# lucidrains/imagen-pytorch

Hardware: AMD Instinct MI355X
Metric: images/sec (64->256 cascade, 1000 steps, bs=8) (higher is better)
Workload: dtype f16; 1 GPU; C3: README unet1 (dim 32, 64^2) + unet2 (dim 32, 256^2, lowres_cond) cascade, 1000 DDPM steps/stage, CFG 3.0, dynamic thresholding, batch 8 per GPU; global_batch=8, parallelism=batch-sharded x1, one RCCL all-gather of final images, batch_schedule=5 whole cascades side by side (one stream each), images_in_flight=40, denoiser_evals_per_image=4000

## Files before the change

imagen-pytorch_amd/_abi.py:

```python
from __future__ import annotations

import ctypes
import os
import re
from typing import Dict

HERE = os.path.dirname(os.path.abspath(__file__))
ROOT = os.path.dirname(HERE)
HEADER = os.path.join(ROOT, "include", "imagen_hip.h")
LIB_PATH = os.environ.get("IMAGEN_LIB_PATH") or os.path.join(HERE, "libimagen_hip.so")

KNOWN_ENV = {"IMAGEN_LIB_PATH", "IMAGEN_TIMING", "IMAGEN_TIME_TABLE", "IMAGEN_TIME_TABLE_MAX_GB", "IMAGEN_CONV_PRO", "IMAGEN_CONV_GEMM",
             "IMAGEN_CONV_SMALL", "IMAGEN_ROWCHAIN", "IMAGEN_EMUL_TESTS", "IMAGEN_BENCH_LANES", "IMAGEN_BENCH_MODE", "IMAGEN_VIDEO_GPU_TESTS"}
_stale = sorted(k for k in os.environ if k.startswith("IMAGEN_") and k not in KNOWN_ENV)
if _stale:
    raise RuntimeError(f"{', '.join(_stale)}: not read by this version (switches of earlier rounds are module constants of imagen_pytorch_amd.ops / "
                       f".engine now: monkeypatch them); known variables: {', '.join(sorted(KNOWN_ENV))}")

_CTYPE = {
    "int32_t": ctypes.c_int32,
    "uint32_t": ctypes.c_uint32,
    "uint8_t": ctypes.c_uint8,
    "float": ctypes.c_float,
}


def _parse_header(path: str):
    text = open(path).read()
    text = re.sub(r"/\*.*?\*/", "", text, flags=re.S)
    text = re.sub(r"//[^\n]*", "", text)
    enums: Dict[str, int] = {}
    for m in re.finditer(r"enum\s*\w*\s*\{(.*?)\}", text, flags=re.S):
        nxt = 0
        for item in m.group(1).split(","):
            item = item.strip()
            if not item:
                continue
            if "=" in item:
                name, val = [s.strip() for s in item.split("=")]
                nxt = int(val, 0)
            else:
                name = item
            enums[name] = nxt
            nxt += 1
    for m in re.finditer(r"#define\s+(IMAGEN_\w+)\s+\(?([0-9x*+ ]+)\)?\s*$", text, flags=re.M):
        try:
            enums[m.group(1)] = int(eval(m.group(2), {}, {}))
        except Exception:
            pass
    structs = {}
    for m in re.finditer(r"typedef\s+struct\s+(\w+)\s*\{(.*?)\}\s*(\w+)\s*;", text, flags=re.S):
        name, body = m.group(3), m.group(2)
        fields = []
        for decl in body.split(";"):
            decl = " ".join(decl.split())
            if not decl:
                continue
            if "*" in decl:
                fname = decl.split("*")[-1].strip()
                fields.append((fname, ctypes.c_void_p))
            else:
                parts = decl.split(" ", 1)
                ctype = _CTYPE[parts[0]]
                for fname in parts[1].split(","):
                    fields.append((fname.strip(), ctype))
        structs[name] = fields
    return enums, structs


ENUMS, _STRUCT_FIELDS = _parse_header(HEADER)


def _make_struct(name, fields):
    return type(name, (ctypes.Structure,), {"_fields_": fields})


STRUCTS = {name: _make_struct(name, fields) for name, fields in _STRUCT_FIELDS.items()}
globals().update(STRUCTS)

OP_STRUCT = {
    ENUMS["IMAGEN_OP_IGEMM"]: STRUCTS["ImagenIgemmParams"],
    ENUMS["IMAGEN_OP_ROWSTAT"]: STRUCTS["ImagenRowstatParams"],
    ENUMS["IMAGEN_OP_ATTENTION"]: STRUCTS["ImagenAttentionParams"],
    ENUMS["IMAGEN_OP_KV_PREP"]: STRUCTS["ImagenKvPrepParams"],
    ENUMS["IMAGEN_OP_QNORM"]: STRUCTS["ImagenQnormParams"],
    ENUMS["IMAGEN_OP_GCA_PARTIAL"]: STRUCTS["ImagenGcaPartialParams"],
    ENUMS["IMAGEN_OP_GCA_FINAL"]: STRUCTS["ImagenGcaFinalParams"],
    ENUMS["IMAGEN_OP_GATE_RESIDUAL"]: STRUCTS["ImagenGateResidualParams"],
    ENUMS["IMAGEN_OP_LN_RESIDUAL"]: STRUCTS["ImagenLnResidualParams"],
    ENUMS["IMAGEN_OP_TIME_EMBED"]: STRUCTS["ImagenTimeEmbedParams"],
    ENUMS["IMAGEN_OP_SCALE_SHIFT"]: STRUCTS["ImagenScaleShiftParams"],
    ENUMS["IMAGEN_OP_PACK_IMAGE"]: STRUCTS["ImagenPackImageParams"],
    ENUMS["IMAGEN_OP_CFG_X0"]: STRUCTS["ImagenCfgX0Params"],
    ENUMS["IMAGEN_OP_QUANTILE"]: STRUCTS["ImagenQuantileParams"],
    ENUMS["IMAGEN_OP_DDPM_UPDATE"]: STRUCTS["ImagenDdpmUpdateParams"],
    ENUMS["IMAGEN_OP_ROWS_COPY"]: STRUCTS["ImagenRowsCopyParams"],
    ENUMS["IMAGEN_OP_MEMSET32"]: STRUCTS["ImagenMemset32Params"],
    ENUMS["IMAGEN_OP_SELECT_ROWS"]: STRUCTS["ImagenSelectRowsParams"],
    ENUMS["IMAGEN_OP_MEAN_ROWS"]: STRUCTS["ImagenMeanRowsParams"],
    ENUMS["IMAGEN_OP_RANDN"]: STRUCTS["ImagenRandnParams"],
    ENUMS["IMAGEN_OP_LOWRES_PREP"]: STRUCTS["ImagenLowresPrepParams"],
    ENUMS["IMAGEN_OP_LINCOMB"]: STRUCTS["ImagenLincombParams"],
    ENUMS["IMAGEN_OP_KV_PREP_MULTI"]: STRUCTS["ImagenKvPrepMultiParams"],
    ENUMS["IMAGEN_OP_TEMPORAL_PEG"]: STRUCTS["ImagenTemporalPegParams"],
    ENUMS["IMAGEN_OP_TEMPORAL_ATTENTION"]: STRUCTS["ImagenTemporalAttentionParams"],
    ENUMS["IMAGEN_OP_ACT_PREP"]: STRUCTS["ImagenActPrepParams"],
    ENUMS["IMAGEN_OP_GCA_TAIL"]: STRUCTS["ImagenGcaTailParams"],
    ENUMS["IMAGEN_OP_STEP_SLICE"]: STRUCTS["ImagenStepSliceParams"],
    ENUMS["IMAGEN_OP_ROWCHAIN"]: STRUCTS["ImagenRowchainParams"],
    ENUMS["IMAGEN_OP_LINEAR_F32"]: STRUCTS["ImagenLinearF32Params"],
    ENUMS["IMAGEN_OP_LINCTX"]: STRUCTS["ImagenLinCtxParams"],
    ENUMS["IMAGEN_OP_LINEAR_XATTN"]: STRUCTS["ImagenLinearXattnParams"],
}
STRUCT_KIND = {v: k for k, v in OP_STRUCT.items()}

EXPORTED_SYMBOLS = [
    "imagen_abi_version", "imagen_last_error", "imagen_sizeof", "imagen_launch", "imagen_plan_run",
    "imagen_igemm_num_configs", "imagen_igemm_config_info", "imagen_igemm_stage_slots", "imagen_igemm_config_family", "imagen_igemm_config_ring", "imagen_igemm_lds_bytes", "imagen_igemm_packed_elems", "imagen_pack_igemm_weights",
    "imagen_graph_begin", "imagen_graph_end", "imagen_graph_launch", "imagen_graph_destroy",
    "imagen_event_create", "imagen_event_record", "imagen_event_elapsed_ms", "imagen_event_destroy",
    "imagen_probe_copy", "imagen_probe_mfma", "imagen_probe_latency", "imagen_probe_launch_chain",
]


class ImagenHipError(RuntimeError):
    pass


_lib = None


def load_library(path: str = LIB_PATH) -> ctypes.CDLL:
    global _lib
    if _lib is not None:
        return _lib
    if not os.path.exists(path):
        raise ImagenHipError(
            f"{path} not found: the HIP extension is the product path and has no fallback. "
            "Build it with `python -c 'import __graft_entry__ as g; g.build()'` (needs hipcc)."
        )
    import torch

    lib = ctypes.CDLL(path)
    for sym in EXPORTED_SYMBOLS:
        if not hasattr(lib, sym):
            raise ImagenHipError(f"{path} does not export {sym}")
    lib.imagen_last_error.restype = ctypes.c_char_p
    lib.imagen_sizeof.restype = ctypes.c_size_t
    lib.imagen_sizeof.argtypes = [ctypes.c_int]
    lib.imagen_launch.argtypes = [ctypes.c_int, ctypes.c_void_p, ctypes.c_size_t, ctypes.c_void_p]
    lib.imagen_plan_run.argtypes = [ctypes.c_void_p, ctypes.c_int, ctypes.c_void_p]
    lib.imagen_igemm_config_info.argtypes = [ctypes.c_int] + [ctypes.POINTER(ctypes.c_int)] * 3
    lib.imagen_igemm_stage_slots.argtypes = [ctypes.c_int] * 3
    lib.imagen_igemm_config_family.argtypes = [ctypes.c_int]
    lib.imagen_igemm_config_ring.argtypes = [ctypes.c_int]
    lib.imagen_igemm_lds_bytes.restype = ctypes.c_long
    lib.imagen_igemm_lds_bytes.argtypes = [ctypes.c_int] * 6
    lib.imagen_igemm_packed_elems.restype = ctypes.c_size_t
    lib.imagen_igemm_packed_elems.argtypes = [ctypes.c_int] * 5
    lib.imagen_pack_igemm_weights.argtypes = [ctypes.c_int, ctypes.c_void_p, ctypes.c_void_p] + [ctypes.c_int] * 5 + [ctypes.c_void_p]
    lib.imagen_graph_begin.argtypes = [ctypes.c_void_p]
    lib.imagen_graph_end.argtypes = [ctypes.c_void_p, ctypes.POINTER(ctypes.c_void_p)]
    lib.imagen_graph_launch.argtypes = [ctypes.c_void_p, ctypes.c_void_p]
    lib.imagen_graph_destroy.argtypes = [ctypes.c_void_p]
    lib.imagen_event_create.argtypes = [ctypes.POINTER(ctypes.c_void_p)]
    lib.imagen_event_record.argtypes = [ctypes.c_void_p, ctypes.c_void_p]
    lib.imagen_event_elapsed_ms.argtypes = [ctypes.c_void_p, ctypes.c_void_p, ctypes.POINTER(ctypes.c_float)]
    lib.imagen_event_destroy.argtypes = [ctypes.c_void_p]
    lib.imagen_probe_copy.argtypes = [ctypes.c_void_p, ctypes.c_void_p, ctypes.c_size_t, ctypes.c_int, ctypes.c_void_p, ctypes.POINTER(ctypes.c_float)]
    lib.imagen_probe_mfma.argtypes = [ctypes.c_int, ctypes.c_int, ctypes.c_void_p, ctypes.c_void_p, ctypes.POINTER(ctypes.c_float)]
    lib.imagen_probe_latency.argtypes = [ctypes.c_void_p, ctypes.c_int, ctypes.c_void_p, ctypes.c_void_p, ctypes.POINTER(ctypes.c_float)]
    lib.imagen_probe_launch_chain.argtypes = [ctypes.c_int, ctypes.c_int, ctypes.c_void_p, ctypes.c_void_p, ctypes.POINTER(ctypes.c_float)]
    if lib.imagen_abi_version() != ENUMS["IMAGEN_ABI_VERSION"]:
        raise ImagenHipError("libimagen_hip.so ABI version does not match include/imagen_hip.h")
    for kind, st in OP_STRUCT.items():
        if lib.imagen_sizeof(kind) != ctypes.sizeof(st):
            raise ImagenHipError(f"struct size mismatch for op kind {kind}: C {lib.imagen_sizeof(kind)} vs ctypes {ctypes.sizeof(st)}")
    _lib = lib
    return lib


def hip_runtime_copies() -> list:
    seen = []
    try:
        with open("/proc/self/maps") as f:
            for line in f:
                if "libamdhip64" in line:
                    path = line.split()[-1]
                    if path not in seen:
                        seen.append(path)
    except OSError:
        pass
    return seen


def check(rc: int, what: str = "") -> None:
    if rc != 0:
        msg = load_library().imagen_last_error().decode(errors="replace")
        raise ImagenHipError(f"{what or 'libimagen_hip'} failed (rc={rc}): {msg}")


class OpRef(ctypes.Structure):
    _fields_ = [("kind", ctypes.c_int32), ("params_bytes", ctypes.c_int32), ("params", ctypes.c_void_p)]
```

imagen-pytorch_amd/build_ext.py:

```python
from __future__ import annotations

import hashlib
import os
import shutil
import subprocess
import sys

HERE = os.path.dirname(os.path.abspath(__file__))
ROOT = os.path.dirname(HERE)
CSRC = os.path.join(HERE, "csrc")
SOURCES = ["igemm.hip", "conv_dma.hip", "conv_stream.hip", "conv_pw.hip", "conv_big.hip", "conv_pro.hip", "conv_gemm.hip", "conv_small.hip", "rowchain.hip", "elementwise.hip", "attention.hip", "sampler.hip", "temporal.hip", "linear_xattn.hip", "codesize.hip", "probe.hip", "capi.hip"]
LIB = os.path.join(HERE, "libimagen_hip.so")
STAMP = os.path.join(HERE, ".libimagen_hip.stamp")


def _torch_lib_dir():
    try:
        import torch
        return os.path.join(os.path.dirname(torch.__file__), "lib")
    except Exception:
        return None


def _digest() -> str:
    h = hashlib.sha256()
    for name in sorted(os.listdir(CSRC)):
        with open(os.path.join(CSRC, name), "rb") as f:
            h.update(name.encode())
            h.update(f.read())
    with open(os.path.join(ROOT, "include", "imagen_hip.h"), "rb") as f:
        h.update(f.read())
    return h.hexdigest()


def build(force: bool = False, verbose: bool = True) -> str:
    digest = _digest()
    if not force and os.path.exists(LIB) and os.path.exists(STAMP) and open(STAMP).read().strip() == digest:
        return LIB
    hipcc = shutil.which("hipcc") or "/opt/rocm/bin/hipcc"
    if not os.path.exists(hipcc):
        raise RuntimeError("hipcc not found: cannot build libimagen_hip.so")
    objs = []
    build_dir = os.path.join(HERE, "build")
    os.makedirs(build_dir, exist_ok=True)
    common = [hipcc, "--offload-arch=gfx950", "-O3", "-std=c++17", "-fPIC", "-I" + os.path.join(ROOT, "include"), "-I" + CSRC]
    procs = []
    for src in SOURCES:
        obj = os.path.join(build_dir, src.replace(".hip", ".o"))
        objs.append(obj)
        procs.append((src, subprocess.Popen(common + ["-c", os.path.join(CSRC, src), "-o", obj],
                                            stdout=subprocess.PIPE, stderr=subprocess.STDOUT)))
    for src, pr in procs:
        out, _ = pr.communicate()
        if pr.returncode != 0:
            raise RuntimeError(f"hipcc failed on {src}:\n{out.decode()}")
        if verbose and out.strip():
            print(out.decode())
    link = [hipcc, "--offload-arch=gfx950", "-shared", "-fPIC", "-o", LIB] + objs
    tl = _torch_lib_dir()
    if tl and os.path.exists(os.path.join(tl, "libamdhip64.so")):
        link += ["-L" + tl, "-Wl,-rpath," + tl]
    link += ["-Wl,-rpath,/opt/rocm/lib"]
    res = subprocess.run(link, stdout=subprocess.PIPE, stderr=subprocess.STDOUT)
    if res.returncode != 0:
        raise RuntimeError("link failed:\n" + res.stdout.decode())
    with open(STAMP, "w") as f:
        f.write(digest)
    if verbose:
        print(f"built {LIB}")
    return LIB


def build_variant(tag: str, defs, sources=None) -> str:
    hipcc = shutil.which("hipcc") or "/opt/rocm/bin/hipcc"
    build_dir = os.path.join(HERE, "build", tag)
    os.makedirs(build_dir, exist_ok=True)
    common = [hipcc, "--offload-arch=gfx950", "-O3", "-std=c++17", "-fPIC", "-I" + os.path.join(ROOT, "include"), "-I" + CSRC] + list(defs)
    procs, objs = [], []
    for src in SOURCES:
        obj = os.path.join(build_dir, src.replace(".hip", ".o"))
        objs.append(obj)
        procs.append((src, subprocess.Popen(common + ["-c", os.path.join(CSRC, src), "-o", obj], stdout=subprocess.PIPE, stderr=subprocess.STDOUT)))
    for src, pr in procs:
        out, _ = pr.communicate()
        if pr.returncode != 0:
            raise RuntimeError(f"hipcc failed on {src}:\n{out.decode()}")
    lib = os.path.join(HERE, f"libimagen_hip_{tag}.so")
    link = [hipcc, "--offload-arch=gfx950", "-shared", "-fPIC", "-o", lib] + objs
    tl = _torch_lib_dir()
    if tl and os.path.exists(os.path.join(tl, "libamdhip64.so")):
        link += ["-L" + tl, "-Wl,-rpath," + tl]
    link += ["-Wl,-rpath,/opt/rocm/lib"]
    res = subprocess.run(link, stdout=subprocess.PIPE, stderr=subprocess.STDOUT)
    if res.returncode != 0:
        raise RuntimeError("link failed:\n" + res.stdout.decode())
    return lib


if __name__ == "__main__":
    build(force="--force" in sys.argv)
```

imagen-pytorch_amd/csrc/conv_families.h:

```cpp
#pragma once
#include "common.h"

int imagen_conv_dma_num_configs();
int imagen_conv_dma_config_info(int idx, int* tile_pixels, int* tile_cout, int* kgroups);
long imagen_conv_dma_lds_bytes(int idx, int KH, int KW, int TH, int TW);
int launch_conv_dma(const ImagenIgemmParams* p, int idx, hipStream_t s);
int imagen_conv_dma_ring(int idx);
int imagen_conv_stream_num_configs();
int imagen_conv_stream_config_info(int idx, int* tile_pixels, int* tile_cout, int* kgroups);
long imagen_conv_stream_lds_bytes(int idx, int KH, int KW, int TH, int TW);
int launch_conv_stream(const ImagenIgemmParams* p, int idx, hipStream_t s);
int imagen_conv_pw_num_configs();
int imagen_conv_pw_config_info(int idx, int* tile_pixels, int* tile_cout, int* kgroups);
long imagen_conv_pw_lds_bytes(int idx, int KH, int KW, int TH, int TW);
int launch_conv_pw(const ImagenIgemmParams* p, int idx, hipStream_t s);
int imagen_conv_big_num_configs();
int imagen_conv_big_config_info(int idx, int* tile_pixels, int* tile_cout, int* kgroups);
long imagen_conv_big_lds_bytes(int idx, int KH, int KW, int TH, int TW);
int launch_conv_big(const ImagenIgemmParams* p, int idx, hipStream_t s);
int imagen_conv_pro_num_configs();
int imagen_conv_pro_config_info(int idx, int* tile_pixels, int* tile_cout, int* kgroups);
long imagen_conv_pro_lds_bytes(int idx, int KH, int KW, int TH, int TW);
int launch_conv_pro(const ImagenIgemmParams* p, int idx, hipStream_t s);
int imagen_conv_gemm_num_configs();
int imagen_conv_gemm_config_info(int idx, int* tile_pixels, int* tile_cout, int* kgroups);
long imagen_conv_gemm_lds_bytes(int idx, int KH, int KW, int TH, int TW);
int launch_conv_gemm(const ImagenIgemmParams* p, int idx, hipStream_t s);
int imagen_conv_small_num_configs();
int imagen_conv_small_config_info(int idx, int* tile_pixels, int* tile_cout, int* kgroups);
long imagen_conv_small_lds_bytes(int idx, int KH, int KW, int TH, int TW);
int launch_conv_small(const ImagenIgemmParams* p, int idx, hipStream_t s);

struct ConvFamily {
  int id;
  int (*num)();
  int (*info)(int idx, int* tile_pixels, int* tile_cout, int* kgroups);
  long (*lds)(int idx, int KH, int KW, int TH, int TW);
  int (*launch)(const ImagenIgemmParams* p, int idx, hipStream_t s);
  int kh, kw;
  int (*ring)(int idx);
};
```

imagen-pytorch_amd/csrc/igemm.hip:

```cpp
#include <algorithm>
#include <cstdio>
#include <cstdlib>
#include <type_traits>
#include <utility>
#include "common.h"
#include "conv_families.h"

namespace {

struct TileCfg { int MI, NI, WM, WN, G; };
constexpr int kBiasLds = 1024;

constexpr int stage_slots(int TP, int G, int KSC) {
  if (KSC == 18 && G == 4) return TP == 64 ? 2 : TP == 128 ? 3 : 6;
  if (KSC == 2 && G == 4) return TP / 64;
  if (KSC == 8 && G == 4) return TP == 64 ? 4 : 6;
  if (KSC == 6 && G == 4) return TP == 64 ? 3 : TP == 128 ? 4 : 5;
  if (KSC == 4 && G == 8) return TP / 32;
  if (KSC == 8 && G == 16) return TP / 16;
  return 4;
}

constexpr TileCfg kCfgs[] = {
    {2, 1, 4, 1, 4},
// ... 603 lines not shown
          if (p.act_out == IMAGEN_ACT_SILU) {
#pragma unroll
            for (int e = 0; e < 4; ++e) v[e] = silu_f(v[e]);
          } else if (p.act_out == IMAGEN_ACT_GELU) {
#pragma unroll
            for (int e = 0; e < 4; ++e) v[e] = gelu_f(v[e]);
          }
          if (p.out_mode == IMAGEN_OUT_NCHW_F32) {
            float* y = reinterpret_cast<float*>(p.y);
#pragma unroll
            for (int e = 0; e < 4; ++e)
              if (co + e < p.Cout) y[((size_t)b * p.Cout + co + e) * (p.OH * p.OW) + op[mi]] = v[e];
            continue;
          }
          if (addend) {
            const f16x4 ad = cur.ar[mi];
            v[0] += (float)ad[0] * cur.g.x; v[1] += (float)ad[1] * cur.g.y; v[2] += (float)ad[2] * cur.g.z; v[3] += (float)ad[3] * cur.g.w;
          } else if (res) {
            const f16x4 rr = cur.ar[mi];
#pragma unroll
            for (int e = 0; e < 4; ++e) v[e] += (float)rr[e];
          }
          f16x4 o;
#pragma unroll
          for (int e = 0; e < 4; ++e) {
            o[e] = (f16)v[e];
            const float r = (float)o[e];
            ssq_px[mi] += r * r;
          }
          outv[ni][q][mi] = o;
        }
      } else {
#pragma unroll
        for (int mi = 0; mi < MI; ++mi) outv[ni][q][mi] = f16x4{};
      }
    });
    prime_weights(n0_next);
    if (wide) {
      f16* y = reinterpret_cast<f16*>(p.y) + (size_t)b * p.bsy;
#pragma unroll
      for (int ni = 0; ni < NI; ++ni)
#pragma unroll
        for (int qp = 0; qp < 2; ++qp) {
          const int cx = n0 + (wn * NI + ni) * 32 + 8 * qp + 16 * half;
#pragma unroll
          for (int mi = 0; mi < MI; ++mi) {
            const imagen_u32x4 v = imagen_pair_quads(outv[ni][qp][mi], outv[ni][qp + 2][mi]);
            if (cx < p.Cout && op[mi] >= 0) *reinterpret_cast<imagen_u32x4*>(y + (size_t)op[mi] * p.ldy + cx) = v;
          }
        }
    } else if (wide_ps) {
      f16* y = reinterpret_cast<f16*>(p.y) + (size_t)b * p.bsy;
      const int Cq = p.Cout >> 2;
#pragma unroll
      for (int ni = 0; ni < NI; ++ni)
#pragma unroll
        for (int qp = 0; qp < 2; ++qp) {
          const int cx = n0 + (wn * NI + ni) * 32 + 8 * qp + 16 * half;
          const int sub = cx / Cq, c = cx - sub * Cq;
#pragma unroll
          for (int mi = 0; mi < MI; ++mi) {
            const imagen_u32x4 v = imagen_pair_quads(outv[ni][qp][mi], outv[ni][qp + 2][mi]);
            const int oy = tc.oy0 + pix_y[mi], ox = tc.ox0 + pix_x[mi];
            const int yy = 2 * oy + (sub >> 1), xx = 2 * ox + (sub & 1);
            if (cx < p.Cout && op[mi] >= 0) *reinterpret_cast<imagen_u32x4*>(y + ((size_t)yy * (2 * p.OW) + xx) * p.ldy + c) = v;
          }
        }
    } else if (p.out_mode != IMAGEN_OUT_NCHW_F32) {
      f16* y = reinterpret_cast<f16*>(p.y);
#pragma unroll
      for (int ni = 0; ni < NI; ++ni)
#pragma unroll
        for (int q = 0; q < 4; ++q) {
          const int co = n0 + (wn * NI + ni) * 32 + 8 * q + 4 * half;
          if (co >= p.Cout) continue;
#pragma unroll
          for (int mi = 0; mi < MI; ++mi) {
            if (op[mi] < 0) continue;
            if (p.out_mode == IMAGEN_OUT_PIXEL_SHUFFLE) {
              const int Cq = p.Cout >> 2;
              const int sub = co / Cq, c = co - sub * Cq;
              const int oy = tc.oy0 + pix_y[mi], ox = tc.ox0 + pix_x[mi];
              const int yy = 2 * oy + (sub >> 1), xx = 2 * ox + (sub & 1);
              *reinterpret_cast<f16x4*>(y + (size_t)b * p.bsy + ((size_t)yy * (2 * p.OW) + xx) * p.ldy + c) = outv[ni][q][mi];
            } else {
              *reinterpret_cast<f16x4*>(y + (size_t)b * p.bsy + (size_t)op[mi] * p.ldy + co) = outv[ni][q][mi];
            }
          }
        }
    }
    }
    if (p.ssq_out) {
#pragma unroll
      for (int mi = 0; mi < MI; ++mi) ssq_px[mi] += __shfl_xor(ssq_px[mi], 32);
      if (WN == 1) {
        if (half == 0) {
#pragma unroll
          for (int mi = 0; mi < MI; ++mi) {
            const int oy = tc.oy0 + pix_y[mi], ox = tc.ox0 + pix_x[mi];
            if (oy < p.OH && ox < p.OW) p.ssq_out[(size_t)b * (p.OH * p.OW) + oy * p.OW + ox] = ssq_px[mi];
          }
        }
      } else {
        if (half == 0) {
#pragma unroll
          for (int mi = 0; mi < MI; ++mi) ep_red[(wm * WN + wn) * PXW + mi * 32 + l31] = ssq_px[mi];
        }
        lds_barrier();
        if (wn == 0 && half == 0) {
#pragma unroll
          for (int mi = 0; mi < MI; ++mi) {
            float tot = 0.0f;
#pragma unroll
            for (int w = 0; w < WN; ++w) tot += ep_red[(wm * WN + w) * PXW + mi * 32 + l31];
            const int oy = tc.oy0 + pix_y[mi], ox = tc.ox0 + pix_x[mi];
            if (oy < p.OH && ox < p.OW) p.ssq_out[(size_t)b * (p.OH * p.OW) + oy * p.OW + ox] = tot;
          }
        }
      }
    }
  };

  TileCoord tc = decode(t_cursor);
  prime_weights(tc.n0);
  unsigned warm_ep = 0;
  if constexpr (GEN) {
    const f16* eop = addend ? addend + (size_t)tc.b * p.bs_add : (res ? res + (size_t)tc.b * p.bs_res : nullptr);
    const int eld = addend ? p.ld_add : p.ld_res;
    if (eop) {
#pragma unroll
      for (int mi = 0; mi < MI; ++mi) {
        const int oy = tc.oy0 + pix_y[mi], ox = tc.ox0 + pix_x[mi];
        const int opx = (oy < p.OH && ox < p.OW) ? oy * p.OW + ox : 0;
#pragma unroll
        for (int ni = 0; ni < NI; ++ni) {
          const int co = min(tc.n0 + (wn * NI + ni) * 32 + 4 * half, p.Cout - 4);
          warm_ep ^= *reinterpret_cast<const volatile unsigned*>(eop + (size_t)opx * eld + co);
        }
      }
      if (addend) warm_ep ^= *reinterpret_cast<const volatile unsigned*>(p.gate + (size_t)tc.b * p.gate_stride + min(tc.n0 + wn * NI * 32 + (lane & 31), p.Cout - 1));
    }
  }
  lds_barrier();
  imagen_code_warm_sink(warm);
  imagen_code_warm_sink(warm_ep);
  int cur = 0;
  while (true) {
    const int t_next = t_cursor + t_step;
    const int n0_next = t_next < t_end ? decode(t_next).n0 : tc.n0;
    for (int chunk = 0; chunk < NC; ++chunk) {
      compute(smem + cur * buf_bytes);
      lds_barrier();
      cur ^= 1;
    }
    epilogue(tc, n0_next);
    if (t_next >= t_end) break;
    zero_acc();
    t_cursor = t_next;
    tc = decode(t_cursor);
  }
}

inline int num_cus() {
  static int n = 0;
  if (n == 0) {
    int dev = 0, v = 0;
    if (hipGetDevice(&dev) == hipSuccess && hipDeviceGetAttribute(&v, hipDeviceAttributeMultiprocessorCount, dev) == hipSuccess && v > 0) n = v;
    else n = 256;
  }
  return n;
}

template <int MI, int NI, int WM, int WN, int G, int KSC, bool GEN>
int launch_gen(const ImagenIgemmParams& p, hipStream_t s);

template <int MI, int NI, int WM, int WN, int G, int KSC>
int launch_ksc(const ImagenIgemmParams& p, hipStream_t s) {
  const bool plain = p.act_out == IMAGEN_ACT_NONE && p.out_mode == IMAGEN_OUT_NHWC && !p.addend && !p.res &&
                     (p.bias == nullptr || p.Cout_pad <= kBiasLds);
  return plain ? launch_gen<MI, NI, WM, WN, G, KSC, false>(p, s) : launch_gen<MI, NI, WM, WN, G, KSC, true>(p, s);
}

template <int MI, int NI, int WM, int WN, int G, int KSC, bool GEN>
int launch_gen(const ImagenIgemmParams& p, hipStream_t s) {
  constexpr int TP = 32 * MI * WM, BN = 32 * NI * WN;
  const int ITW = (p.TW - 1) * p.stride + p.KW, ITH = (p.TH - 1) * p.stride + p.KH;
  const int IT = ITH * ITW;
  IMAGEN_CHECK(p.TH * p.TW == TP, "igemm: tile %dx%d does not match cfg %d (%d pixels)", p.TH, p.TW, p.cfg, TP);
  IMAGEN_CHECK(IT * G <= stage_slots(TP, G, KSC) * 256, "igemm: halo tile too large (%d px x %d groups > %d staging slots)", IT, G,
               stage_slots(TP, G, KSC));
  IMAGEN_CHECK(p.Cout_pad % BN == 0, "igemm: Cout_pad %d not a multiple of %d", p.Cout_pad, BN);
  IMAGEN_CHECK(p.Cin_pad % (8 * G) == 0, "igemm: Cin_pad %d not a multiple of %d", p.Cin_pad, 8 * G);
  IMAGEN_CHECK(p.C1 % 8 == 0 && p.C2 % 8 == 0 && p.ld1 % 8 == 0 && (p.x2 == nullptr || p.ld2 % 8 == 0),
               "igemm: channel counts / strides must be multiples of 8 (C1=%d C2=%d ld1=%d ld2=%d)", p.C1, p.C2, p.ld1, p.ld2);
  IMAGEN_CHECK(p.out_mode == IMAGEN_OUT_NCHW_F32 || p.Cout % 4 == 0, "igemm: Cout %d must be a multiple of 4", p.Cout);
  IMAGEN_CHECK(p.out_mode != IMAGEN_OUT_PIXEL_SHUFFLE || p.Cout % 16 == 0, "igemm: pixel-shuffle needs Cout %% 16 == 0");
  IMAGEN_CHECK(!p.post_pa || (p.post_ps && p.out_mode == IMAGEN_OUT_NHWC && p.Cout <= BN && !p.addend && !p.res && !p.ssq_out &&
                              p.act_out == IMAGEN_ACT_NONE && p.Cout % 4 == 0),
               "igemm: post_pa needs post_ps, a plain NHWC output and one workgroup covering all %d output channels (tile has %d)", p.Cout, BN);
  IMAGEN_CHECK(!(p.addend && p.res), "igemm: addend and residual are mutually exclusive");
  IMAGEN_CHECK(!p.ssq_out || (p.out_mode == IMAGEN_OUT_NHWC && p.Cout <= BN),
               "igemm: ssq_out needs NHWC output and one workgroup covering all %d output channels (tile has %d)", p.Cout, BN);
  const size_t lds = (size_t)2 * IT * Geo<G>::PS + (size_t)(4 * 32 * MI + kBiasLds) * sizeof(float) + 16;
  IMAGEN_CHECK(lds <= 160 * 1024, "igemm: LDS tile %zu bytes too large", lds);
  auto kern = igemm_kernel<MI, NI, WM, WN, G, KSC, GEN>;
  static bool attr_done[16] = {};
  int dev = 0;
  (void)hipGetDevice(&dev);
  if (dev < 0 || dev >= 16 || !attr_done[dev]) {
    hipError_t e = hipFuncSetAttribute(reinterpret_cast<const void*>(kern), hipFuncAttributeMaxDynamicSharedMemorySize, 160 * 1024);
    if (e != hipSuccess) { imagen_set_error("igemm: hipFuncSetAttribute: %s", hipGetErrorString(e)); return (int)e; }
    if (dev >= 0 && dev < 16) attr_done[dev] = true;
  }
  const int tilesX = (p.OW + p.TW - 1) / p.TW, tilesY = (p.OH + p.TH - 1) / p.TH;
  const int total = p.B * tilesX * tilesY * ((p.Cout + BN - 1) / BN);
  static size_t occ_lds = 0;
  static int occ_blocks = 0;
  if (occ_blocks == 0 || occ_lds != lds) {
    int nb = 0;
    if (hipOccupancyMaxActiveBlocksPerMultiprocessor(&nb, reinterpret_cast<const void*>(kern), 512, lds) != hipSuccess || nb < 1) nb = 1;
    occ_blocks = nb;
    occ_lds = lds;
  }
  const int resident = std::max(8, num_cus() * occ_blocks / 8 * 8);
  int gx;
  if (total <= resident) {
    gx = total;
  } else {
    const int rounds = (total + resident - 1) / resident;
    gx = (total + rounds - 1) / rounds;
    gx = std::min(resident, (gx + 7) / 8 * 8);
  }
  static const unsigned code_q = [] {
    char name[160];
    snprintf(name, sizeof(name), "_ZN12_GLOBAL__N_112igemm_kernelILi%dELi%dELi%dELi%dELi%dELi%dELb%dEEEv17ImagenIgemmParams", MI, NI, WM, WN, G, KSC,
             GEN ? 1 : 0);
    return std::min(imagen_kernel_code_bytes(name) >> 8, 0xffffu);
  }();
  ImagenIgemmParams q = p;
  q.launcher_word = (int)code_q;
  hipLaunchKernelGGL(kern, dim3(gx), dim3(512), lds, s, q);
  return imagen_hip_status("igemm launch");
}

template <int MI, int NI, int WM, int WN, int G>
int launch_cfg(const ImagenIgemmParams& p, hipStream_t s) {
  const int ks = (p.KH * p.KW * G + 1) / 2;
  if (G == 4) {
    if (ks == 18) return launch_ksc<MI, NI, WM, WN, G, (G == 4 ? 18 : 0)>(p, s);
    if (ks == 2) return launch_ksc<MI, NI, WM, WN, G, (G == 4 ? 2 : 0)>(p, s);
    if (ks == 8) return launch_ksc<MI, NI, WM, WN, G, (G == 4 ? 8 : 0)>(p, s);
    if (ks == 6) return launch_ksc<MI, NI, WM, WN, G, (G == 4 ? 6 : 0)>(p, s);
  }
  if (G == 8 && ks == 4) return launch_ksc<MI, NI, WM, WN, G, (G == 8 ? 4 : 0)>(p, s);
  if (G == 16 && ks == 8) return launch_ksc<MI, NI, WM, WN, G, (G == 16 ? 8 : 0)>(p, s);
  if (G == 1 && ks == 113) return launch_ksc<MI, NI, WM, WN, G, (G == 1 ? 113 : 0)>(p, s);
  return launch_ksc<MI, NI, WM, WN, G, 0>(p, s);
}

}

static const ConvFamily kFamilies[] = {
    {2, imagen_conv_dma_num_configs, imagen_conv_dma_config_info, imagen_conv_dma_lds_bytes, launch_conv_dma, 3, 3, imagen_conv_dma_ring},
    {3, imagen_conv_stream_num_configs, imagen_conv_stream_config_info, imagen_conv_stream_lds_bytes, launch_conv_stream, 3, 3, nullptr},
    {4, imagen_conv_pw_num_configs, imagen_conv_pw_config_info, imagen_conv_pw_lds_bytes, launch_conv_pw, 1, 1, nullptr},
    {5, imagen_conv_big_num_configs, imagen_conv_big_config_info, imagen_conv_big_lds_bytes, launch_conv_big, 3, 3, nullptr},
    {6, imagen_conv_pro_num_configs, imagen_conv_pro_config_info, imagen_conv_pro_lds_bytes, launch_conv_pro, 3, 3, nullptr},
    {7, imagen_conv_gemm_num_configs, imagen_conv_gemm_config_info, imagen_conv_gemm_lds_bytes, launch_conv_gemm, 1, 1, nullptr},
    {8, imagen_conv_small_num_configs, imagen_conv_small_config_info, imagen_conv_small_lds_bytes, launch_conv_small, 3, 3, nullptr},
};

struct CfgRef {
  const ConvFamily* fam;
  int idx;
};

static CfgRef cfg_ref(int cfg) {
  CfgRef r = {nullptr, cfg};
  int base = kNumCfgs;
  for (const ConvFamily& f : kFamilies) {
    if (cfg < base) break;
    r = {&f, cfg - base};
    base += f.num();
  }
  return r;
}

static int cfg_end() {
  int n = kNumCfgs;
  for (const ConvFamily& f : kFamilies) n += f.num();
  return n;
}

int launch_igemm(const ImagenIgemmParams* pp, hipStream_t s) {
  const ImagenIgemmParams& p = *pp;
  IMAGEN_CHECK(p.cfg >= 0 && p.cfg < cfg_end(), "igemm: bad cfg %d", p.cfg);
  IMAGEN_CHECK(p.x1 && p.w && p.y, "igemm: null x1/w/y");
  IMAGEN_CHECK(!p.addend || p.gate, "igemm: addend requires gate");
  IMAGEN_CHECK(p.cfg >= kNumCfgs || (p.TW > 0 && (p.TW & (p.TW - 1)) == 0), "igemm: tile width %d is not a power of two", p.TW);
  IMAGEN_CHECK(!p.pad_x1 || p.cfg < kNumCfgs, "igemm: pad_x1 (an x padding of its own) is implemented by kernel family 0 only (cfg %d)", p.cfg);
  IMAGEN_CHECK(p.pad_x1 >= 0, "igemm: pad_x1 %d", p.pad_x1);
  IMAGEN_CHECK(!p.gca_part || p.cfg >= kNumCfgs, "igemm: gca_part is implemented by the kernel families 2, 5, 7 and 8 only (cfg %d)", p.cfg);
  const CfgRef r = cfg_ref(p.cfg);
  if (r.fam) return r.fam->launch(pp, r.idx, s);
  switch (p.cfg) {
    case 0: return launch_cfg<2, 1, 4, 1, 4>(p, s);
    case 1: return launch_cfg<4, 1, 1, 4, 4>(p, s);
    case 2: return launch_cfg<4, 1, 2, 2, 4>(p, s);
    case 3: return launch_cfg<2, 1, 1, 4, 4>(p, s);
    case 4: return launch_cfg<1, 1, 4, 1, 4>(p, s);
    case 5: return launch_cfg<2, 1, 4, 1, 1>(p, s);
    case 6: return launch_cfg<1, 1, 2, 2, 4>(p, s);
    case 7: return launch_cfg<1, 2, 2, 2, 1>(p, s);
    case 8: return launch_cfg<1, 1, 2, 2, 1>(p, s);
    case 9: return launch_cfg<1, 1, 4, 1, 1>(p, s);
    case 10: return launch_cfg<2, 1, 1, 4, 16>(p, s);
    case 11: return launch_cfg<4, 1, 1, 4, 8>(p, s);
    case 12: return launch_cfg<1, 1, 2, 2, 16>(p, s);
    case 13: return launch_cfg<1, 1, 4, 1, 8>(p, s);
    case 14: return launch_cfg<2, 1, 1, 4, 8>(p, s);
    case 15: return launch_cfg<1, 1, 2, 2, 8>(p, s);
  }
  return -1;
}

extern "C" int imagen_igemm_num_configs(void) { return cfg_end(); }

extern "C" int imagen_igemm_config_family(int cfg) {
  if (cfg < 0 || cfg >= imagen_igemm_num_configs()) return -1;
  const CfgRef r = cfg_ref(cfg);
  return r.fam ? r.fam->id : 0;
}

extern "C" int imagen_igemm_config_ring(int cfg) {
  const CfgRef r = cfg_ref(cfg);
  return r.fam && r.fam->ring ? r.fam->ring(r.idx) : 0;
}

extern "C" int imagen_igemm_config_info(int cfg, int* tile_pixels, int* tile_cout, int* kgroups) {
  const CfgRef r = cfg_ref(cfg);
  if (r.fam) return r.fam->info(r.idx, tile_pixels, tile_cout, kgroups);
  if (cfg < 0 || cfg >= kNumCfgs) return -1;
  const TileCfg& c = kCfgs[cfg];
  if (tile_pixels) *tile_pixels = 32 * c.MI * c.WM;
  if (tile_cout) *tile_cout = 32 * c.NI * c.WN;
  if (kgroups) *kgroups = c.G;
  return 0;
}

static constexpr int ksc_of(int G, int ks) {
  if (G == 4 && (ks == 18 || ks == 2 || ks == 8 || ks == 6)) return ks;
  if (G == 8 && ks == 4) return ks;
  if (G == 16 && ks == 8) return ks;
  if (G == 1 && ks == 113) return ks;
  return 0;
}

extern "C" int imagen_igemm_stage_slots(int cfg, int KH, int KW) {
  const CfgRef r = cfg_ref(cfg);
  if (r.fam) return (KH == r.fam->kh && KW == r.fam->kw) ? 1 << 20 : 0;
  if (cfg < 0 || cfg >= kNumCfgs || KH < 1 || KW < 1) return -1;
  const TileCfg& c = kCfgs[cfg];
  return stage_slots(32 * c.MI * c.WM, c.G, ksc_of(c.G, (KH * KW * c.G + 1) / 2));
}

extern "C" long imagen_igemm_lds_bytes(int cfg, int KH, int KW, int stride, int TH, int TW) {
  const CfgRef r = cfg_ref(cfg);
  if (r.fam) return stride == 1 ? r.fam->lds(r.idx, KH, KW, TH, TW) : -1;
  if (cfg < 0 || KH < 1 || KW < 1 || TH < 1 || TW < 1) return -1;
  const TileCfg& c = kCfgs[cfg];
  if (TH * TW != 32 * c.MI * c.WM) return -1;
  const int IT = ((TH - 1) * stride + KH) * ((TW - 1) * stride + KW);
  if (IT * c.G > imagen_igemm_stage_slots(cfg, KH, KW) * 256) return -1;
  const long PS = c.G == 1 ? 16 : c.G * 16 + 16;
  const long lds = 2 * IT * PS + (long)(4 * 32 * c.MI + kBiasLds) * (long)sizeof(float) + 16;
  return lds <= 160 * 1024 ? lds : -1;
}

static inline int round_up(int v, int m) { return (v + m - 1) / m * m; }
constexpr int kTailSteps = 16;

extern "C" size_t imagen_igemm_packed_elems(int G, int Cin, int Cout_pad, int KH, int KW) {
  if (G != 1 && G != 2 && G != 4 && G != 8 && G != 16) return 0;
  const int KC = 8 * G;
  const int NC = round_up(Cin, KC) / KC;
  const int KGP = ((KH * KW * G + 1) / 2) * 2;
  return (size_t)(NC * KGP + kTailSteps * 2) * Cout_pad * 8;
}

extern "C" int imagen_pack_igemm_weights(int G, const float* w_in, const float* in_scale, int Cin, int Cout, int Cout_pad,
                                         int KH, int KW, uint16_t* w_out) {
  if (G != 1 && G != 2 && G != 4 && G != 8 && G != 16) { imagen_set_error("pack: bad G %d", G); return -1; }
  if (Cout_pad < Cout || Cout_pad % 32) { imagen_set_error("pack: bad Cout_pad %d", Cout_pad); return -1; }
  const int KC = 8 * G;
  const int Cin_pad = round_up(Cin, KC);
  const int NC = Cin_pad / KC, ntap = KH * KW;
  const int KGP = ((ntap * G + 1) / 2) * 2;
  const size_t total = (size_t)(NC * KGP + kTailSteps * 2) * Cout_pad * 8;
  f16* out = reinterpret_cast<f16*>(w_out);
  for (size_t i = 0; i < total; ++i) out[i] = (f16)0.0f;
  for (int chunk = 0; chunk < NC; ++chunk)
    for (int tap = 0; tap < ntap; ++tap)
      for (int cg = 0; cg < G; ++cg)
        for (int co = 0; co < Cout; ++co)
          for (int j = 0; j < 8; ++j) {
            const int ci = chunk * KC + cg * 8 + j;
            if (ci >= Cin) continue;
            float v = w_in[((size_t)co * Cin + ci) * ntap + tap];
            if (in_scale) v *= in_scale[ci];
            out[((size_t)(chunk * KGP + tap * G + cg) * Cout_pad + co) * 8 + j] = (f16)v;
          }
  return 0;
}
```

Before: 1.382 images/s.

## Add dedicated narrow-output 3x3 conv kernel for final output convs

Adds a specialized direct 3x3 convolution kernel for layers with at most 4 output channels and at most 64 input channels, such as the final image-output conv. Each lane computes one output column over R rows and uses fdot2 on f16 pairs, with weights staged in LDS. The igemm dispatcher routes qualifying raw-input, plain fp32-NCHW-store convs to it by default, with an env switch to disable. The aim is to avoid the wasted MMA tile width of the general implicit-GEMM kernels when Cout is tiny. The risk is lower compute efficiency than MMA paths when the layer is large.

```diff
diff --git a/imagen-pytorch_amd/_abi.py b/imagen-pytorch_amd/_abi.py
--- a/imagen-pytorch_amd/_abi.py
+++ b/imagen-pytorch_amd/_abi.py
@@ -11,7 +11,7 @@
 LIB_PATH = os.environ.get("IMAGEN_LIB_PATH") or os.path.join(HERE, "libimagen_hip.so")
 
 KNOWN_ENV = {"IMAGEN_LIB_PATH", "IMAGEN_TIMING", "IMAGEN_TIME_TABLE", "IMAGEN_TIME_TABLE_MAX_GB", "IMAGEN_CONV_PRO", "IMAGEN_CONV_GEMM",
-             "IMAGEN_CONV_SMALL", "IMAGEN_ROWCHAIN", "IMAGEN_EMUL_TESTS", "IMAGEN_BENCH_LANES", "IMAGEN_BENCH_MODE", "IMAGEN_VIDEO_GPU_TESTS"}
+             "IMAGEN_CONV_SMALL", "IMAGEN_CONV_NARROW", "IMAGEN_ROWCHAIN", "IMAGEN_EMUL_TESTS", "IMAGEN_BENCH_LANES", "IMAGEN_BENCH_MODE", "IMAGEN_VIDEO_GPU_TESTS"}
 _stale = sorted(k for k in os.environ if k.startswith("IMAGEN_") and k not in KNOWN_ENV)
 if _stale:
     raise RuntimeError(f"{', '.join(_stale)}: not read by this version (switches of earlier rounds are module constants of imagen_pytorch_amd.ops / "
diff --git a/imagen-pytorch_amd/build_ext.py b/imagen-pytorch_amd/build_ext.py
--- a/imagen-pytorch_amd/build_ext.py
+++ b/imagen-pytorch_amd/build_ext.py
@@ -9,7 +9,7 @@
 HERE = os.path.dirname(os.path.abspath(__file__))
 ROOT = os.path.dirname(HERE)
 CSRC = os.path.join(HERE, "csrc")
-SOURCES = ["igemm.hip", "conv_dma.hip", "conv_stream.hip", "conv_pw.hip", "conv_big.hip", "conv_pro.hip", "conv_gemm.hip", "conv_small.hip", "rowchain.hip", "elementwise.hip", "attention.hip", "sampler.hip", "temporal.hip", "linear_xattn.hip", "codesize.hip", "probe.hip", "capi.hip"]
+SOURCES = ["igemm.hip", "conv_dma.hip", "conv_stream.hip", "conv_pw.hip", "conv_big.hip", "conv_pro.hip", "conv_gemm.hip", "conv_small.hip", "conv_narrow.hip", "rowchain.hip", "elementwise.hip", "attention.hip", "sampler.hip", "temporal.hip", "linear_xattn.hip", "codesize.hip", "probe.hip", "capi.hip"]
 LIB = os.path.join(HERE, "libimagen_hip.so")
 STAMP = os.path.join(HERE, ".libimagen_hip.stamp")
 
diff --git a/imagen-pytorch_amd/csrc/conv_families.h b/imagen-pytorch_amd/csrc/conv_families.h
--- a/imagen-pytorch_amd/csrc/conv_families.h
+++ b/imagen-pytorch_amd/csrc/conv_families.h
@@ -30,6 +30,8 @@
 int imagen_conv_small_config_info(int idx, int* tile_pixels, int* tile_cout, int* kgroups);
 long imagen_conv_small_lds_bytes(int idx, int KH, int KW, int TH, int TW);
 int launch_conv_small(const ImagenIgemmParams* p, int idx, hipStream_t s);
+bool imagen_conv_narrow_takes(const ImagenIgemmParams* p, int G);
+int launch_conv_narrow(const ImagenIgemmParams* p, int G, hipStream_t s);
 
 struct ConvFamily {
   int id;
diff --git a/imagen-pytorch_amd/csrc/conv_narrow.hip b/imagen-pytorch_amd/csrc/conv_narrow.hip
--- /dev/null
+++ b/imagen-pytorch_amd/csrc/conv_narrow.hip
@@ -0,0 +1,171 @@
+#include <algorithm>
+#include <type_traits>
+#include "conv_families.h"
+
+namespace {
+
+constexpr int kMaxGroups = 8;
+constexpr int kMaxCout = 4;
+
+__device__ __forceinline__ float dot8(const uint4& a, const uint4& w, float c) {
+  const f16x8 av = __builtin_bit_cast(f16x8, a), wv = __builtin_bit_cast(f16x8, w);
+#ifdef IMAGEN_EMUL
+#pragma unroll
+  for (int j = 0; j < 8; j += 2) c += (float)av[j] * (float)wv[j] + (float)av[j + 1] * (float)wv[j + 1];
+#else
+#pragma unroll
+  for (int j = 0; j < 8; j += 2) c = __builtin_amdgcn_fdot2(f16x2{av[j], av[j + 1]}, f16x2{wv[j], wv[j + 1]}, c, false);
+#endif
+  return c;
+}
+
+template <int NCO, int R>
+__global__ __launch_bounds__(256, 4) void conv_narrow_kernel(const ImagenIgemmParams p, const int G) {
+  __shared__ uint4 wl[kMaxGroups * 9 * NCO];
+  const int tid = threadIdx.x, lane = tid & 63;
+  const int wave = __builtin_amdgcn_readfirstlane(tid >> 6), nw = blockDim.x >> 6;
+  const int g1 = p.C1 >> 3, ngrp = (p.C1 + p.C2) >> 3;
+  {
+    const uint4* wsrc = reinterpret_cast<const uint4*>(p.w);
+    const int KGP = (9 * G + 1) & ~1;
+    for (int i = tid; i < ngrp * 9 * NCO; i += blockDim.x) {
+      const int co = i % NCO, t = (i / NCO) % 9, grp = i / (NCO * 9);
+      const int chunk = grp / G, cg = grp - chunk * G;
+      wl[i] = wsrc[(size_t)(chunk * KGP + t * G + cg) * p.Cout_pad + co];
+    }
+  }
+  __syncthreads();
+  const int ox = blockIdx.x * 64 + lane;
+  const int oy0 = (blockIdx.y * nw + wave) * R;
+  const int b = blockIdx.z;
+  if (oy0 >= p.OH) return;
+
+  float acc[R][NCO];
+#pragma unroll
+  for (int o = 0; o < R; ++o)
+#pragma unroll
+    for (int co = 0; co < NCO; ++co) acc[o][co] = 0.0f;
+
+  const char* x1 = reinterpret_cast<const char*>(reinterpret_cast<const f16*>(p.x1) + (size_t)b * p.bs1);
+  const char* x2 = reinterpret_cast<const char*>(reinterpret_cast<const f16*>(p.x2) + (size_t)b * p.bs2);
+  const int ld1_s = __builtin_amdgcn_readfirstlane(p.ld1), ld2_s = __builtin_amdgcn_readfirstlane(p.ld2);
+  const int oxc = min(ox, p.W - 1);
+  auto run = [&](auto inner) __attribute__((always_inline)) {
+  constexpr bool INNER = decltype(inner)::value;
+  for (int c0 = 0; c0 < ngrp; c0 += 4) {
+    const int c1 = min(c0 + 4, ngrp);
+#pragma unroll
+    for (int dx = 0; dx < 3; ++dx) {
+      const int ix = oxc + dx - 1;
+      const bool col_ok = dx == 1 || (ix >= 0 && ix < p.W);
+      const int ixc = col_ok ? ix : oxc;
+      unsigned pix[R + 2];
+#pragma unroll
+      for (int r = 0; r < R + 2; ++r) pix[r] = (unsigned)(min(max(oy0 + r - 1, 0), p.H - 1) * p.W + ixc);
+      auto load_rows = [&](int grp, uint4 (&a)[R + 2]) __attribute__((always_inline)) {
+        const bool from1 = grp < g1;
+        const char* src = from1 ? x1 + grp * 16 : x2 + (grp - g1) * 16;
+        const unsigned ld = (unsigned)(from1 ? ld1_s : ld2_s);
+#pragma unroll
+        for (int r = 0; r < R + 2; ++r) {
+          const int iy = oy0 + r - 1;
+          a[r] = make_uint4(0u, 0u, 0u, 0u);
+          if (INNER || (iy >= 0 && iy < p.H)) {
+            const uint4 v = *reinterpret_cast<const uint4*>(src + (size_t)(pix[r] * ld * 2u));
+            a[r] = col_ok ? v : make_uint4(0u, 0u, 0u, 0u);
+          }
+        }
+      };
+      auto mul_rows = [&](int grp, const uint4 (&a)[R + 2]) __attribute__((always_inline)) {
+        float part[R][NCO];
+#pragma unroll
+        for (int o = 0; o < R; ++o)
+#pragma unroll
+          for (int co = 0; co < NCO; ++co) part[o][co] = 0.0f;
+#pragma unroll
+        for (int dy = 0; dy < 3; ++dy)
+#pragma unroll
+          for (int co = 0; co < NCO; ++co) {
+            const uint4 w = wl[(grp * 9 + dy * 3 + dx) * NCO + co];
+#pragma unroll
+            for (int o = 0; o < R; ++o) part[o][co] = dot8(a[o + dy], w, part[o][co]);
+          }
+#pragma unroll
+        for (int o = 0; o < R; ++o)
+#pragma unroll
+          for (int co = 0; co < NCO; ++co) acc[o][co] += part[o][co];
+      };
+      uint4 a0[R + 2], a1[R + 2];
+      load_rows(c0, a0);
+      for (int grp = c0; grp < c1; grp += 2) {
+        if (grp + 1 < c1) load_rows(grp + 1, a1);
+        mul_rows(grp, a0);
+        if (grp + 1 < c1) {
+          if (grp + 2 < c1) load_rows(grp + 2, a0);
+          mul_rows(grp + 1, a1);
+        }
+      }
+    }
+  }
+  };
+  if (oy0 >= 1 && oy0 + R + 1 <= p.H) run(std::true_type{});
+  else run(std::false_type{});
+
+  if (ox >= p.OW) return;
+  float* y = reinterpret_cast<float*>(p.y);
+  const size_t plane = (size_t)p.OH * p.OW;
+#pragma unroll
+  for (int co = 0; co < NCO; ++co) {
+    const float bias = p.bias ? p.bias[co] : 0.0f;
+#pragma unroll
+    for (int o = 0; o < R; ++o) {
+      const int oy = oy0 + o;
+      if (oy < p.OH) y[((size_t)b * NCO + co) * plane + (size_t)oy * p.OW + ox] = acc[o][co] + bias;
+    }
+  }
+}
+
+template <int NCO, int R>
+int launch_nr(const ImagenIgemmParams& p, int G, hipStream_t s) {
+  const long waves = (long)p.B * ((p.OW + 63) / 64) * ((p.OH + R - 1) / R);
+  const int nw = waves >= 4096 ? 4 : 1;
+  const dim3 grid((p.OW + 63) / 64, (p.OH + R * nw - 1) / (R * nw), p.B);
+  hipLaunchKernelGGL((conv_narrow_kernel<NCO, R>), grid, dim3(64 * nw), 0, s, p, G);
+  return imagen_hip_status("conv_narrow launch");
+}
+
+template <int NCO>
+int launch_n(const ImagenIgemmParams& p, int G, hipStream_t s) {
+  const long waves4 = (long)p.B * ((p.OW + 63) / 64) * ((p.OH + 3) / 4);
+  return waves4 >= 1024 ? launch_nr<NCO, 4>(p, G, s) : launch_nr<NCO, 1>(p, G, s);
+}
+
+}
+
+bool imagen_conv_narrow_takes(const ImagenIgemmParams* pp, int G) {
+  const ImagenIgemmParams& p = *pp;
+  const bool geom = p.KH == 3 && p.KW == 3 && p.stride == 1 && p.pad == 1 && p.pad_x1 == 0 && p.OH == p.H && p.OW == p.W && p.B >= 1 && p.B <= 65535 &&
+                    p.H >= 1 && p.W >= 1 && (long)p.H * p.W < (1L << 24) && (long)p.H * p.W * std::max(p.ld1, p.ld2) < (1L << 31);
+  const bool chans = p.Cout >= 1 && p.Cout <= kMaxCout && p.Cout_pad >= p.Cout && p.C1 >= 8 && p.C1 % 8 == 0 && p.C2 >= 0 && p.C2 % 8 == 0 &&
+                     (p.C2 == 0 || p.x2 != nullptr) && p.C1 + p.C2 <= 8 * kMaxGroups && p.C1 + p.C2 <= p.Cin_pad &&
+                     (G == 1 || G == 2 || G == 4 || G == 8 || G == 16) && p.Cin_pad % (8 * G) == 0;
+  const bool aligned = p.ld1 % 8 == 0 && p.bs1 % 8 == 0 && ((size_t)p.x1 & 15) == 0 && ((size_t)p.w & 15) == 0 &&
+                       (p.C2 == 0 || (p.ld2 % 8 == 0 && p.bs2 % 8 == 0 && ((size_t)p.x2 & 15) == 0));
+  const bool raw = !p.mu && !p.rs && !p.pa && !p.ps && !p.ssq_a && !p.ssq_b && p.act_in == IMAGEN_ACT_NONE;
+  const bool plain = p.out_mode == IMAGEN_OUT_NCHW_F32 && p.act_out == IMAGEN_ACT_NONE && !p.addend && !p.res && !p.ssq_out && !p.post_pa &&
+                     !p.post_ps && !p.gca_part;
+  return geom && chans && aligned && raw && plain;
+}
+
+int launch_conv_narrow(const ImagenIgemmParams* pp, int G, hipStream_t s) {
+  const ImagenIgemmParams& p = *pp;
+  IMAGEN_CHECK(imagen_conv_narrow_takes(pp, G),
+               "conv_narrow: 3x3 s1 p1, Cout <= %d, C1 + C2 <= %d in 16-byte aligned multiples of 8, raw inputs, bias + fp32-NCHW store only "
+               "(k%dx%d s%d p%d Cout %d C %d+%d out_mode %d)", kMaxCout, 8 * kMaxGroups, p.KH, p.KW, p.stride, p.pad, p.Cout, p.C1, p.C2, p.out_mode);
+  switch (p.Cout) {
+    case 1: return launch_n<1>(p, G, s);
+    case 2: return launch_n<2>(p, G, s);
+    case 3: return launch_n<3>(p, G, s);
+    default: return launch_n<4>(p, G, s);
+  }
+}
diff --git a/imagen-pytorch_amd/csrc/igemm.hip b/imagen-pytorch_amd/csrc/igemm.hip
--- a/imagen-pytorch_amd/csrc/igemm.hip
+++ b/imagen-pytorch_amd/csrc/igemm.hip
@@ -929,6 +929,13 @@
   IMAGEN_CHECK(p.pad_x1 >= 0, "igemm: pad_x1 %d", p.pad_x1);
   IMAGEN_CHECK(!p.gca_part || p.cfg >= kNumCfgs, "igemm: gca_part is implemented by the kernel families 2, 5, 7 and 8 only (cfg %d)", p.cfg);
   const CfgRef r = cfg_ref(p.cfg);
+  if (!r.fam || r.fam->kh == 3) {
+    int G = 0;
+    if (imagen_igemm_config_info(p.cfg, nullptr, nullptr, &G) == 0 && imagen_conv_narrow_takes(pp, G)) {
+      const char* sw = getenv("IMAGEN_CONV_NARROW");
+      if (!(sw && sw[0] == '0' && sw[1] == 0)) return launch_conv_narrow(pp, G, s);
+    }
+  }
   if (r.fam) return r.fam->launch(pp, r.idx, s);
   switch (p.cfg) {
     case 0: return launch_cfg<2, 1, 4, 1, 4>(p, s);
```

Result: no change. 1.377 images/s (-0.4%).
